# naver/panst3r

Hardware: AMD Instinct MI355X
Metric: frames/sec (whole node), N-view 512px panoptic inference (higher is better)
Workload: dtype f16

## Files before the change

### include/panst3r_hip.h

```cpp
#ifndef PANST3R_HIP_H
#define PANST3R_HIP_H
#include <stdint.h>
#ifdef __cplusplus
extern "C" {
#endif

#define PST_ABI_VERSION 20

#define PST_BF16 0
#define PST_F32  1
#define PST_F16  2
#define PST_X3H  4

int pst_abi_version(void);
const char* pst_last_error(void);

typedef struct pst_gemm_params {
  const void* A;  int64_t lda;
  const void* W;  int64_t ldw;
  void* C;        int64_t ldc;
  int32_t M, N, K;
  const float* bias;
  const float* gamma;
  const float* res;  int64_t ldr;
  int32_t res_mod;
  int32_t act;
  int32_t out_fp32;
  int32_t trans_out;
  int32_t grp_in, grp_out, grp_off;
  int32_t ps_p, ps_c, ps_h, ps_w;
  int32_t conv_c, conv_h, conv_w;
  const void* zeros;
  const int32_t* rope_pos; const float* rope_cs; int32_t rope_hd;
  int32_t rope_npos;
  int32_t res_bf16;
  int32_t kernel;
  int32_t batch;
  int64_t a_bs, w_bs, c_bs, bias_bs;
  int32_t dtype16;
  void* xcopy; int64_t ldxc;
  float* stats_out; int32_t stats_ld;
  const float* ln_stats; int32_t ln_groups; const float* ln_colsum; float ln_eps;
  int32_t x3_block;
} pst_gemm_params;

int pst_gemm(const pst_gemm_params* p, void* stream);
const char* pst_gemm_variant(const pst_gemm_params* p);
int pst_gemm_pair(const pst_gemm_params* a, const pst_gemm_params* b, void* stream);
const char* pst_gemm_pair_variant(const pst_gemm_params* a, const pst_gemm_params* b);
#define PST_TUNE_G256_PP 3
#define PST_TUNE_PAIR 4
#define PST_TUNE_DEEP_RING 8
#define PST_TUNE_PAIR_ATTN 7
#define PST_TUNE_ATTN_XCD 9
#define PST_TUNE_CUS 10
#define PST_TUNE_PAIR_DELAY 6
#define PST_TUNE_DEPHASE 11
#define PST_TUNE_PAIR_RES 5
int pst_tune(int knob, int value);

int pst_mask_head_supported(int Q, int P, int C);
int pst_mask_head(const void* E, int64_t lde, const void* F, int64_t f_view_stride, float* out, int64_t out_view_stride, int nviews, int Q, int P, int C,
                  int dtype16, void* stream);

typedef struct pst_attn_params {
  const void* Q;  int64_t q_bs, q_hs, q_rs;
  const void* K;  int64_t k_bs, k_hs, k_rs;
  const void* Vt; int64_t v_bs, v_hs, v_ds;
  void* O;        int64_t o_bs, o_hs, o_rs;
  const uint8_t* mask; int64_t m_bs, m_rs;
  int32_t B, H, Nq, Nk, hd;
  float scale;
  const void* zeros;
  int32_t nsplit;
  void* ws; int64_t ws_bytes;
  int32_t dtype16;
  int32_t prescaled;
} pst_attn_params;

int64_t pst_attn_workspace_bytes(int B, int H, int Nq, int hd, int nsplit);

int pst_attn_fwd(const pst_attn_params* p, void* stream);
const char* pst_attn_variant(const pst_attn_params* p);
int pst_attn_pair(const pst_attn_params* a, const pst_attn_params* b, void* stream);
const char* pst_attn_pair_variant(const pst_attn_params* a, const pst_attn_params* b);

int pst_layernorm(const void* x, int64_t ldx, int in_fp32, void* y, int64_t ldy, int out_fp32,
                  const float* gamma, const float* beta, int rows, int D, float eps,
                  int grp_in, int grp_out, int grp_off, void* stream);
int pst_layernorm_add(const void* x, int64_t ldx, int in_fp32, const float* add, int64_t ld_add, void* y, int64_t ldy,
                      int out_fp32, const float* gamma, const float* beta, int rows, int D, float eps,
                      int grp_in, int grp_out, int grp_off, void* stream);

int pst_token_embed(const int32_t* ids, int B, int L, const float* tok, int vocab, const float* pos, int npos, int D, float* out, int64_t ldo,
                    int32_t* status, void* stream);

int pst_rowstats(const void* x, int64_t ldx, int x_type, void* xcopy, int64_t ldxc, float* stats, int stats_ld, int rows, int D, int dtype16,
                 void* stream);

int pst_layernorm_add_batch(const void* x, int64_t ldx, int in_fp32, const float* add, int64_t ld_add, void* y, int64_t ldy,
                            int out_fp32, const float* gamma, const float* beta, int rows, int D, float eps,
                            int grp_in, int grp_out, int grp_off, int nbatch, int64_t x_bs, int64_t y_bs, int64_t w_bs,
                            void* stream);

int pst_split3(const float* x, int64_t ldx, void* out, int64_t ldo, int rows, int K, int dtype16, void* stream);

int pst_split_operand(const float* x, int64_t ldx, void* out, int64_t ldo, int rows, int K, int Kpad, int side, int dtype16, void* stream);
int pst_split2(const float* x, int64_t ldx, void* hi, void* lo, int64_t ldo, int rows, int K, int transpose, int dtype16, void* stream);
int pst_transpose_f32(const float* x, int64_t ldx, float* y, int64_t ldy, int rows, int cols, void* stream);
int pst_rope2d_split(const float* x, int64_t ld, const int32_t* pos, const float* cs, void* hi, void* lo, int64_t ldo, int rows, int nheads, int hd, int dtype16,
                     void* stream);
int pst_attn_x3(const pst_attn_params* p, const void* Q_lo, const void* K_lo, const void* Vt_lo, int out_type, int64_t out_block, void* stream);
const char* pst_attn_x3_variant(const pst_attn_params* p);

int pst_rope2d(void* x, int64_t ld, const int32_t* pos, const float* cs, int rows, int nheads, int hd, int dtype16,
               void* stream);

int pst_patchify(const float* img, void* out, int64_t ld, int nimg, int C, int H, int W, int p, int dtype16, void* stream);
int pst_dino_preprocess(const float* img, float* out, int nimg, int H, int W, int Ho, int Wo, void* stream);

int pst_image_prepare(const uint8_t* src, int Hs, int Ws, float* dst, int Hr, int Wr, int top, int left, int H, int W, void* stream);
int pst_patch_rows(const float* img, void* enc, int64_t ld_enc, void* dino, int64_t ld_dino, int nimg, int H, int W, int p_enc, int p_dino,
                   int dino_transposed, int dtype16, void* stream);

int pst_add_cast(const void* a, int64_t lda, int a_fp32, const void* b, int64_t ldb, int b_fp32, int b_mod,
                 void* y, int64_t ldy, int y_fp32, int rows, int D, void* stream);
int pst_l2norm_rows(const float* x, int64_t ldx, void* y, int64_t ldy, int rows, int D, float eps, int dtype16, void* stream);

int pst_mean4(const void* F, void* Fm, int nimg, int Hm, int Wm, int C, int dtype16, void* stream);
int pst_resize_bilinear(const void* F, void* Fd, int nimg, int Hs, int Ws, int Hd, int Wd, int C, int dtype16, void* stream);
int pst_attn_mask_from_logits(const float* logits, int64_t ldl, uint8_t* mask, int64_t ldm, int Q, int Nk,
                              void* stream);

#define PST_STATS_BLOCKS 128
int pst_loftup_guidance_gn(const float* img, const float* biases, const float* gamma, const float* beta, float eps,
                           float* scratch, float* stats, void* y, int64_t ldy, int nimg, int H, int W, int nf, int dtype16,
                           const float* mm_ext, void* stream);
int pst_loftup_minmax(const float* img, float* mm, int nimg, int H, int W, void* stream);
int pst_minmax_merge(const float* mm, const int32_t* scope, float* out, int nviews, void* stream);
int pst_groupnorm_stats(const void* x, int64_t ldx, int x_fp32, float* stats, int nimg, int P, int C, int G,
                        void* stream);
int pst_groupnorm_apply(const void* x, int64_t ldx, int x_fp32, const float* stats, const float* gamma,
                        const float* beta, void* y, int64_t ldy, int nimg, int P, int C, int G, float eps, int relu,
                        int dtype16, void* stream);
int pst_loftup_lr_pe(const float* biases, void* out, int64_t ld, int col0, int nimg, int h, int w, int dtype16, void* stream);

int pst_pp_scores(const float* logits, int Q, int Ncls, float cls_threshold, float temperature, float* scores,
                  int* labels, int* keep, void* stream);
int pst_pp_scores_softmax(const float* logits, int Q, int Ncls, float cls_threshold, float* scores, int* labels, int* keep, void* stream);
int pst_pp_sigmoid(const float* logits, const int* keep, float* probs, int Q, int P, void* stream);
int pst_pp_argmax(const float* probs, const float* scores, const int* keep, int Q, int Hm, int Wm, int H, int W,
                  float mask_threshold, int* best_q, float* best_m, int* cnt_orig, int* cnt_mask, void* stream);
int pst_pp_argmax_logits(const float* logits, const float* scores, const int* keep, int Q, int Hm, int Wm, int H, int W,
                         float mask_threshold, int* best_q, float* best_m, int* cnt_orig, int* cnt_mask, void* stream);
int pst_pp_select(const int* keep, int* cnt_orig, int* cnt_mask, int Q, double overlap_threshold, int* keep_out,
                  int* seg_id, void* stream);
int pst_pp_finalize(const int* best_q, const float* best_m, const int* seg_id, int n, float mask_threshold,
                    float void_confidence, int* pan, float* conf, void* stream);

int pst_qubo_upsample(const float* logits, float* probs, int Q, int hm, int wm, int H, int W, void* stream);
int64_t pst_qubo_workspace_floats(int Q, int64_t P);
int pst_qubo_overlap(const float* probs, int Q, int64_t P, float* ws, double* Wacc, void* stream);
int pst_qubo_argmax(const float* probs, const int* sel, int nsel, int64_t P, float* conf, int* inst, void* stream);

int pst_pointmap_activate(const float* raw, float* pts3d, float* pts3d_local, float* conf, int64_t npix, int mode, void* stream);
int pst_focal_weiszfeld(const float* pts3d_local, const float* pp, float* focal, int nviews, int H, int W, int iters, void* stream);
int pst_rigid_moments(const float* x, const float* y, const float* conf, double* out, int nviews, int npix, float weight_offset, void* stream);

int pst_retrieval_select(const float* x, int64_t ldx, const int32_t* in_off, const int32_t* out_off, int nviews, int maxT, int D, float* out, int64_t ldo,
                         int32_t* sel_idx, void* stream);
int pst_retrieval_assign(const void* x3, int64_t ldx, const void* c3, int64_t ldc, const float* cnorm, int n, int k, int K3, int m, int nsplit,
                         float* ws_dist, int32_t* ws_ids, int32_t* ids, float* dist, int dtype16, void* stream);
int pst_retrieval_aggregate(const float* x, int64_t ldx, const float* cent, int64_t ldc, const int32_t* member, const int32_t* gstart, const int32_t* gword,
                            int ngroups, int D, float* sums, uint32_t* bits, void* stream);
int pst_retrieval_scores(const int32_t* q_off, const int32_t* q_word, const uint32_t* q_bits, const int32_t* db_off, const int32_t* db_word,
                         const uint32_t* db_bits, int nq_views, int ndb_views, int max_q, int D, float alpha, float tau, float* S, void* stream);

typedef struct pst_cloud_view {
  const float* conf;
  const float* pts3d;
  const float* pts3d_local;
  const float* img;
  const int32_t* pan;
  int64_t offset;
  int32_t npix;
  int32_t first_wg;
  float c2w[12];
} pst_cloud_view;

int pst_cloud_count(const pst_cloud_view* views, int nviews, int nwg, float thr, int32_t* counts, void* stream);
int pst_cloud_scan(const int32_t* counts, int n, int32_t* base, void* stream);
int pst_cloud_compact(const pst_cloud_view* views, int nviews, int nwg, float thr, const int32_t* base, const float* colors, int ncolors, float w1, float w2,
                      float* points, float* points_local, float* rgb, int32_t* pan, float* colors_out, int64_t* index, void* stream);
int pst_cloud_segment_median(const float* points_local, const int32_t* pan, const int32_t* m_ptr, int64_t max_points, const int32_t* id2row, int ntab, int nseg,
                             int32_t* hist, uint32_t* prefix, int32_t* rank, int32_t* nan_cnt, int32_t* count, float* median, void* stream);

int pst_voxel_insert(const float* points, int64_t M, float inv, uint64_t* keys, int64_t capacity, int32_t* first, int32_t* point_slot, int32_t* status,
                     int merge, void* stream);
int pst_voxel_count(const int32_t* point_slot, const int32_t* first, int64_t M, int32_t* counts, void* stream);
int pst_voxel_rank(const int32_t* point_slot, const int32_t* first, int64_t M, const int32_t* base, int32_t* slot_rank, int32_t* first_row, void* stream);
int pst_voxel_accumulate(const float* points, const float* rgb, const int32_t* pan, int64_t M, float inv, const int32_t* point_slot,
                         const int32_t* slot_rank, const int32_t* id2row, int ntab, int32_t* cnt, uint64_t* sums, uint64_t* pair_keys, int32_t* pair_cnt,
                         int64_t capacity, int32_t* point_voxel, int32_t* status, int merge, void* stream);
int pst_voxel_vote(const uint64_t* pair_keys, const int32_t* pair_cnt, int64_t capacity, uint64_t* best, void* stream);
int pst_voxel_emit(const float* points, const int64_t* index, const int32_t* first_row, const int32_t* mv_ptr, int64_t max_voxels, float inv,
                   double voxel_size, const int32_t* cnt, const uint64_t* sums, const uint64_t* best, const float* colors, int ncolors, float w1, float w2,
                   float* out_points, float* out_rgb, int32_t* out_pan, float* out_colors, int32_t* out_votes, int64_t* out_first, void* stream);

#define PST_VCC_FULL 1
#define PST_VCC_DUPLICATE 2
#define PST_VCC_RANGE 4
// ... 110 lines not shown
```

### panst3r_amd/csrc/gemm.hip

```cpp
#include "common.h"
#include "../../include/panst3r_hip.h"

namespace pst {

int launch_gemm256(const pst_gemm_params& p, hipStream_t s);
int launch_gemm256p(const pst_gemm_params& p, hipStream_t s, int cus);
int gemm256p_pair_split(const pst_gemm_params& a, const pst_gemm_params& b, int cus, double separate_us, double* pair_us);
double gemm256p_single_us(const pst_gemm_params& p, int cus);
int launch_gemm256p_pair(const pst_gemm_params& a, const pst_gemm_params& b, hipStream_t s, int cus, int g0);
bool gemm256_persistent_ok(const pst_gemm_params& p);
int gemm256_persistent_class(const pst_gemm_params& p);
int gemm_f32_validate(const pst_gemm_params& p);
int launch_gemm_f32(const pst_gemm_params& p, hipStream_t s);
int rowstream_class(const pst_gemm_params& p);
int launch_rowstream(const pst_gemm_params& p, hipStream_t s, int cus);

constexpr int BK = 64;
constexpr int GROUP_M = 8;

template <int F>
__device__ __forceinline__ int perm_row(int row) {
  const int sub = row / (16 * F), rho = row - sub * (16 * F);
  const int f = rho >> 4, g = (rho >> 2) & 3, r = rho & 3;
  return sub * (16 * F) + g * (4 * F) + 4 * f + r;
// ... 323 lines not shown
    if (p.grp_in > 0) { quot = rem / p.grp_in; rem -= quot * p.grp_in; }
#pragma unroll
    for (int it = 0; it < BM / 8; ++it) {
      const int r = tid / nchf + it * rstepf;
      const int m = m0 + r;
      resv[it] = make_float4(0.f, 0.f, 0.f, 0.f);
      if (r < BM && m < p.M && nf < p.N) {
        const int orow = p.grp_in > 0 ? quot * p.grp_out + p.grp_off + rem : m;
        resv[it] = *(const float4*)(p.res + (int64_t)(p.res_mod > 0 ? (m % p.res_mod) : orow) * p.ldr + nf);
      }
      rem += rstepf;
      if (p.grp_in > 0) {
        while (rem >= p.grp_in) { rem -= p.grp_in; ++quot; }
      }
    }
  }
  if (TRANS) {
    bf16_t* Ct = (bf16_t*)p.C;
#pragma unroll
    for (int j = 0; j < FN; ++j) {
      const int n = n0 + wc * (16 * FN) + j * 16 + l16;
      if (n >= p.N) continue;
      const float b = p.bias ? p.bias[n] : 0.f;
      const int mb = m0 + wr * (16 * FM) + g * (4 * FM);
      bf16_t* dst = Ct + (int64_t)n * p.ldc + mb;
      const float cs = p.ln_stats ? p.ln_colsum[n] : 0.f;
      float v[4 * FM];
#pragma unroll
      for (int i = 0; i < FM; ++i)
#pragma unroll
        for (int r = 0; r < 4; ++r) {
          const float2 st = p.ln_stats ? lnst[wr * (16 * FM) + g * (4 * FM) + 4 * i + r] : make_float2(1.f, 0.f);
          float x = fmaf(acc[i][j][r], st.x, fmaf(st.y, cs, b));
          if (p.act == 2) x = fmaxf(x, 0.f);
          v[4 * i + r] = x;
        }
      if (p.act == 1) {
#pragma unroll
        for (int i = 0; i < FM; ++i) gelu_erf4(*(float (*)[4])(v + 4 * i));
      }
      if (mb + 4 * FM <= p.M && (((uintptr_t)dst) & 15) == 0) {
#pragma unroll
        for (int q = 0; q < FM / 2; ++q)
          *(uint4*)(dst + 8 * q) = make_uint4(H16<F16>::pack(v[8 * q], v[8 * q + 1]), H16<F16>::pack(v[8 * q + 2], v[8 * q + 3]),
                                              H16<F16>::pack(v[8 * q + 4], v[8 * q + 5]), H16<F16>::pack(v[8 * q + 6], v[8 * q + 7]));
      } else if (mb + 4 * FM <= p.M) {
#pragma unroll
        for (int q = 0; q < FM; ++q)
          *(uint2*)(dst + 4 * q) = make_uint2(H16<F16>::pack(v[4 * q], v[4 * q + 1]), H16<F16>::pack(v[4 * q + 2], v[4 * q + 3]));
      } else {
        for (int r = 0; r < 4 * FM && mb + r < p.M; ++r) dst[r] = H16<F16>::from_f(v[r]);
      }
    }
    return;
  }

  const bool f32o = p.out_fp32 != 0;
  const int pitch = BN * (f32o ? 4 : 2);
  const int nch = pitch >> 4;
  __syncthreads();
  {
    const int cb = wc * (16 * FN) + g * (4 * FN);
    float4 bias4[FN], gam4[FN], cs4[FN];
#pragma unroll
    for (int j = 0; j < FN; ++j) {
      const int n = min(n0 + cb + 4 * j, p.N - 4);
      bias4[j] = p.bias ? *(const float4*)(p.bias + n) : make_float4(0.f, 0.f, 0.f, 0.f);
      gam4[j] = p.gamma ? *(const float4*)(p.gamma + n) : make_float4(1.f, 1.f, 1.f, 1.f);
      cs4[j] = p.ln_stats ? *(const float4*)(p.ln_colsum + n) : make_float4(0.f, 0.f, 0.f, 0.f);
    }
    float2 lns[FM];
#pragma unroll
    for (int i = 0; i < FM; ++i) lns[i] = p.ln_stats ? lnst[wr * (16 * FM) + i * 16 + l16] : make_float2(1.f, 0.f);
#pragma unroll
    for (int i = 0; i < FM; ++i) {
      const int r = wr * (16 * FM) + i * 16 + l16;
      char* rowp = smem + r * pitch;
      const int key = r & (nch - 1);
#pragma unroll
      for (int j = 0; j < FN; ++j) {
        float v[4] = {fmaf(acc[i][j][0], lns[i].x, fmaf(lns[i].y, cs4[j].x, bias4[j].x)), fmaf(acc[i][j][1], lns[i].x, fmaf(lns[i].y, cs4[j].y, bias4[j].y)),
                      fmaf(acc[i][j][2], lns[i].x, fmaf(lns[i].y, cs4[j].z, bias4[j].z)), fmaf(acc[i][j][3], lns[i].x, fmaf(lns[i].y, cs4[j].w, bias4[j].w))};
        if (p.act == 1) {
          gelu_erf4(v);
        } else if (p.act == 2) {
#pragma unroll
          for (int q = 0; q < 4; ++q) v[q] = fmaxf(v[q], 0.f);
        }
        v[0] *= gam4[j].x; v[1] *= gam4[j].y; v[2] *= gam4[j].z; v[3] *= gam4[j].w;
        const int col = cb + 4 * j;
        if (f32o) *(float4*)(rowp + ((((col >> 2) ^ key)) << 4)) = make_float4(v[0], v[1], v[2], v[3]);
        else *(uint2*)(rowp + ((((col >> 3) ^ key)) << 4) + ((col & 4) << 1)) = make_uint2(H16<F16>::pack(v[0], v[1]), H16<F16>::pack(v[2], v[3]));
      }
    }
  }
  __syncthreads();
  if (f32o) row_phase<BM, BN, true, F16>(p, smem, tid, m0, n0, resv);
  else row_phase<BM, BN, false, F16>(p, smem, tid, m0, n0, resv);
}

static int g_cu_budget = 0;
static int num_cus() {
  if (g_cu_budget > 0) return g_cu_budget;
  static int cus = 0;
  if (cus == 0) {
    int dev = 0;
    hipDeviceProp_t prop;
    if (hipGetDevice(&dev) == hipSuccess && hipGetDeviceProperties(&prop, dev) == hipSuccess) cus = prop.multiProcessorCount;
    if (cus <= 0) cus = 256;
  }
  return cus;
}

template <int FM, int FN, bool TRANS, int NST, bool F16>
__global__ __launch_bounds__(256, 2) void gemm_kernel(const pst_gemm_params p, const int ntiles, const int tiles_m, const int tiles_n) {
  gemm_tile<FM, FN, TRANS, NST, F16>(p, ntiles, tiles_m, tiles_n, blockIdx.x, blockIdx.y);
}

template <int FM, int FN, int NST, bool F16>
__global__ __launch_bounds__(256, 2) void gemm_pair_kernel(const pst_gemm_params pa, const int na, const int tma, const int tna,
                                                           const pst_gemm_params pb, const int nb, const int tmb, const int tnb) {
  if ((int)blockIdx.x < na) gemm_tile<FM, FN, false, NST, F16>(pa, na, tma, tna, blockIdx.x, 0);
  else gemm_tile<FM, FN, true, NST, F16>(pb, nb, tmb, tnb, (int)blockIdx.x - na, 0);
}

template <int FM, int FN, int NST, bool F16>
static int launch_pair_t(const pst_gemm_params& a, const pst_gemm_params& b, hipStream_t s) {
  constexpr int BM = 32 * FM, BN = 32 * FN;
  const int tma = (a.M + BM - 1) / BM, tna = (a.N + BN - 1) / BN, tmb = (b.M + BM - 1) / BM, tnb = (b.N + BN - 1) / BN;
  const size_t lds = NST * (BM + BN) * 128 + BM * sizeof(float2);
  hipLaunchKernelGGL((gemm_pair_kernel<FM, FN, NST, F16>), dim3(tma * tna + tmb * tnb), dim3(256), lds, s, a, tma * tna, tma, tna, b, tmb * tnb, tmb, tnb);
  return check_launch("gemm_pair");
}

template <int FM, int FN, bool TRANS, int NST, bool F16>
static int launch_t(const pst_gemm_params& p, hipStream_t s) {
  constexpr int BM = 32 * FM, BN = 32 * FN;
  const int tiles_m = (p.M + BM - 1) / BM, tiles_n = (p.N + BN - 1) / BN;
  const int tiles = tiles_m * tiles_n;
  const size_t lds = NST * (BM + BN) * 128 + BM * sizeof(float2);
  if constexpr (NST > 4) {
    static unsigned long long attr_seen = 0;
    once_per_device(attr_seen, [] { (void)hipFuncSetAttribute((const void*)gemm_kernel<FM, FN, TRANS, NST, F16>, hipFuncAttributeMaxDynamicSharedMemorySize, NST * (BM + BN) * 128 + BM * (int)sizeof(float2)); });
  }
  hipLaunchKernelGGL((gemm_kernel<FM, FN, TRANS, NST, F16>), dim3(tiles, p.batch > 1 ? p.batch : 1), dim3(256), lds, s, p, tiles, tiles_m, tiles_n);
  return check_launch("gemm");
}

template <int FM, int FN, bool TRANS, int NST>
static int launch(const pst_gemm_params& p, hipStream_t s) {
  return p.dtype16 == DT_F16 ? launch_t<FM, FN, TRANS, NST, true>(p, s) : launch_t<FM, FN, TRANS, NST, false>(p, s);
}

}

static int gemm_validate(const pst_gemm_params* pp) {
  using namespace pst;
  if (!pp) { set_error("gemm: null params"); return PST_EINVAL; }
  const pst_gemm_params& p = *pp;
  if (p.dtype16 == DT_F32) {
    if (p.M <= 0 || p.N <= 0 || p.K <= 0 || !p.A || !p.W || !p.C) { set_error("gemm: bad shape / null operand"); return PST_EINVAL; }
    if (p.kernel != 0) { set_error("gemm (fp32 operands): kernel must be 0"); return PST_EINVAL; }
    return pst::gemm_f32_validate(p);
  }
  if (p.dtype16 != DT_BF16 && p.dtype16 != DT_F16) { set_error("gemm: dtype16 must be PST_BF16, PST_F16 or PST_F32"); return PST_EINVAL; }
  if (p.act < 0 || p.act > 2) {
    set_error("gemm: act %d not available with 16-bit operands (0 none, 1 GELU(erf), 2 ReLU; 3 = GELU(tanh) needs fp32 operands)", p.act); return PST_EINVAL;
  }
  if (p.kernel != 0 && p.kernel != 128 && p.kernel != 256) { set_error("gemm: kernel must be 0 (auto), 128 or 256"); return PST_EINVAL; }
  if (p.kernel == 256 && (p.conv_c > 0 || (p.trans_out && pst::gemm256_persistent_class(p) != 3))) {
    set_error("gemm: the 256x256 kernel has no conv mode, and trans_out only in its persistent class (16-bit, ldc %% 8 == 0, N %% 64 == 0)"); return PST_EINVAL;
  }
  if (p.M <= 0 || p.N <= 0 || p.K <= 0) { set_error("gemm: bad shape M=%d N=%d K=%d", p.M, p.N, p.K); return PST_EINVAL; }
  if (p.K % 64 || p.N % 4) { set_error("gemm: need K%%64==0 and N%%4==0 (K=%d N=%d)", p.K, p.N); return PST_EINVAL; }
  if (!p.A || !p.W || !p.C) { set_error("gemm: null operand"); return PST_EINVAL; }
  if ((((uintptr_t)p.A | (uintptr_t)p.W) & 15) || ((uintptr_t)p.C & (p.out_fp32 ? 15 : 7))) {
    set_error("gemm: A/W must be 16-byte aligned, C 8-byte (bf16) / 16-byte (fp32) aligned"); return PST_EINVAL;
  }
  if ((p.ldw % 8) || (p.conv_c == 0 && (p.lda % 8))) { set_error("gemm: lda/ldw must be multiples of 8"); return PST_EINVAL; }
  if (p.conv_c > 0 && (p.conv_c % 64 || p.K != 9 * p.conv_c || !p.zeros || p.M % (p.conv_h * p.conv_w))) {
    set_error("gemm: bad conv mode (conv_c=%d K=%d)", p.conv_c, p.K); return PST_EINVAL;
  }
  if (p.ps_p > 0 && ((p.ps_p * p.ps_c) % 4 || p.N != p.ps_p * p.ps_p * p.ps_c || p.M % (p.ps_h * p.ps_w) || p.res || p.grp_in)) {
    set_error("gemm: bad pixel-shuffle store (p=%d c=%d N=%d)", p.ps_p, p.ps_c, p.N); return PST_EINVAL;
  }
  if (p.trans_out && (p.out_fp32 || p.res || p.gamma || p.grp_in || p.ps_p || (p.ldc % 4))) {
    set_error("gemm: trans_out supports bf16 + bias/act only, ldc%%4==0"); return PST_EINVAL;
  }
  if (!p.trans_out && !p.ps_p && (p.ldc % 4)) { set_error("gemm: ldc must be a multiple of 4"); return PST_EINVAL; }
  if (p.rope_hd != 0 && (p.rope_hd != 64 || p.out_fp32 || p.trans_out || p.ps_p || p.N % 64 || !p.rope_pos || !p.rope_cs || p.res)) {
    set_error("gemm: fused RoPE needs head dim 64, bf16 plain output, N%%64==0, no residual"); return PST_EINVAL;
  }
  if (p.res && (p.ldr % (p.res_bf16 ? 8 : 4))) { set_error("gemm: ldr must be a multiple of 4 (fp32) / 8 (bf16)"); return PST_EINVAL; }
  if (p.res && p.res_bf16 && ((uintptr_t)p.res & 15)) { set_error("gemm: bf16 residual must be 16-byte aligned"); return PST_EINVAL; }
  if ((p.stats_out || p.xcopy) && (p.N % 64 || p.ps_p || p.trans_out || p.res_mod || p.batch > 1 || (p.stats_out && p.stats_ld < p.N / 64) ||
                                   (p.xcopy && (!p.out_fp32 || p.ldxc % 4 || ((uintptr_t)p.xcopy & 7))))) {
    set_error("gemm: LayerNorm-fold producer outputs need a plain row-major store with N%%64==0 (xcopy: fp32 C only)"); return PST_EINVAL;
  }
  if (p.ln_stats && (!p.ln_colsum || p.ln_groups <= 0 || p.conv_c || p.batch > 1 || !(p.ln_eps > 0.f))) {
    set_error("gemm: LayerNorm-fold consumer needs ln_colsum, ln_groups > 0, ln_eps > 0 (no conv / batch mode)"); return PST_EINVAL;
  }
  if (p.x3_block && (!p.out_fp32 || p.dtype16 != DT_F16 || p.x3_block < p.N || p.x3_block % 4 || p.ldc < 3 * (int64_t)p.x3_block || p.ldc % 4 || p.ps_p || p.trans_out || p.xcopy ||
                     p.stats_out || p.batch > 1 || ((uintptr_t)p.C & 7))) {
    set_error("gemm: the split store (x3_block) needs out_fp32, f16 operands, x3_block >= N, ldc >= 3 x3_block, a plain row-major store"); return PST_EINVAL;
  }
  if (p.batch > 1 && (p.gamma || p.res || p.conv_c || p.rope_hd || p.ps_p || p.grp_in || p.kernel == 256 || p.batch > 65535 ||
                      (p.a_bs | p.w_bs | p.c_bs) % 8 || p.bias_bs % 4)) {
    set_error("gemm: strided batch supports bias/act/trans_out only, strides multiples of 8 elements (batch=%d)", p.batch); return PST_EINVAL;
  }
  return PST_OK;
}

static int g_deep_ring = 4;
namespace pst { int gemm256_pp(int set); int gemm256p_dephase(int set); int gemm256p_pair_delay(int set); int attn_pair_enable(int set); int attn_xcd_order(int set); }

static int gemm_choice(const pst_gemm_params& p) {
  const long big_tiles = (long)((p.M + 127) / 128) * ((p.N + 127) / 128) * (p.batch > 1 ? p.batch : 1);
  const bool small = p.kernel == 0 && big_tiles < (p.K >= 2048 ? 176 : 256);
  const long tiles256 = (long)((p.M + 255) / 256) * ((p.N + 255) / 256);
  const bool fits32 = (int64_t)p.M * p.lda < (1ll << 31) && (int64_t)p.N * p.ldw < (1ll << 31);
  const bool one_round = tiles256 >= 176 && tiles256 <= 256;
  if (p.trans_out) {
    const bool p3 = pst::gemm256_persistent_class(p) == 3 && fits32 && p.batch <= 1 && (p.kernel == 256 || (p.kernel == 0 && (tiles256 >= 384 || one_round) && p.K >= 512));
    return p3 ? 2 : (small ? 0 : 1);
  }
  const bool shape256 = p.N % 256 == 0 && p.K >= 1024 && (p.N >= 2048 || p.K >= 2048) && tiles256 >= 3 * 256 - 64;
  const int pclass = pst::gemm256_persistent_class(p);
  const bool shape256p = (tiles256 >= 384 || one_round) && ((pclass == 1 && p.K >= 512) || (pclass == 2 && (p.K >= 2048 || (p.K >= 768 && tiles256 <= 512))));
  if (p.conv_c == 0 && fits32 && p.batch <= 1 && (p.kernel == 256 || (p.kernel == 0 && (shape256 || shape256p)))) return 2;
  return small ? 0 : 1;
}

extern "C" int pst_gemm(const pst_gemm_params* pp, void* stream) {
  using namespace pst;
  if (int rc = gemm_validate(pp)) return rc;
  const pst_gemm_params& p = *pp;
  hipStream_t s = (hipStream_t)stream;
  if (p.dtype16 == DT_F32) return launch_gemm_f32(p, s);
  if (rowstream_class(p)) return launch_rowstream(p, s, num_cus());
  const int c = gemm_choice(p);
  if (c == 2) return gemm256_persistent_ok(p) ? launch_gemm256p(p, s, num_cus()) : launch_gemm256(p, s);
  if (p.trans_out) return c == 0 ? launch<2, 2, true, 4>(p, s) : launch<4, 4, true, 2>(p, s);
  if (c == 0 && g_deep_ring > 4 && p.batch <= 1) {
    const long tiles = (long)((p.M + 63) / 64) * ((p.N + 63) / 64);
    if (tiles <= num_cus() && p.K >= 512) return g_deep_ring >= 8 ? launch<2, 2, false, 8>(p, s) : launch<2, 2, false, 6>(p, s);
  }
  return c == 0 ? launch<2, 2, false, 4>(p, s) : launch<4, 4, false, 2>(p, s);
}

static bool pair_fusable(const pst_gemm_params& a, const pst_gemm_params& b) {
  using namespace pst;
  if (a.dtype16 == DT_F32 || a.dtype16 != b.dtype16 || a.trans_out || !b.trans_out || a.batch > 1 || b.batch > 1 || a.kernel || b.kernel) return false;
  if (rowstream_class(a) || rowstream_class(b)) return false;
  return gemm_choice(a) == 0 && gemm_choice(b) == 0;
}

static int g_pair_res = 1;
static int g_pair = 1;
static int pair_split_256p(const pst_gemm_params& a, const pst_gemm_params& b) {
  using namespace pst;
  if (!g_pair || a.dtype16 == DT_F32 || a.dtype16 != b.dtype16 || a.batch > 1 || b.batch > 1 || a.kernel || b.kernel) return 0;
  if (rowstream_class(a) || rowstream_class(b)) return 0;
  const int cus = num_cus();
  double sep = 0.0;
  const pst_gemm_params* ps[2] = {&a, &b};
  for (const pst_gemm_params* p : ps) {
    const bool fits32 = (int64_t)p->M * p->lda < (1ll << 31) && (int64_t)p->N * p->ldw < (1ll << 31);
    if (gemm_choice(*p) == 2 && gemm256_persistent_ok(*p)) { sep += gemm256p_single_us(*p, cus); continue; }
    const long tiles256 = (long)((p->M + 255) / 256) * ((p->N + 255) / 256);
    if (!(g_pair_res && gemm256_persistent_class(*p) == 2 && fits32 && p->conv_c == 0 && p->K >= 1024 && tiles256 >= 128)) return 0;
    sep += 2.0 * p->M * p->N * p->K / 470e6;
  }
  return gemm256p_pair_split(a, b, cus, sep, nullptr);
}

extern "C" int pst_gemm_pair(const pst_gemm_params* pa, const pst_gemm_params* pb, void* stream) {
  using namespace pst;
  if (int rc = gemm_validate(pa)) return rc;
  if (int rc = gemm_validate(pb)) return rc;
  hipStream_t s = (hipStream_t)stream;
  if (const int g0 = pair_split_256p(*pa, *pb)) return launch_gemm256p_pair(*pa, *pb, s, num_cus(), g0);
  if (!pair_fusable(*pa, *pb)) {
    if (int rc = pst_gemm(pa, stream)) return rc;
    return pst_gemm(pb, stream);
  }
  return pa->dtype16 == DT_F16 ? launch_pair_t<2, 2, 4, true>(*pa, *pb, s) : launch_pair_t<2, 2, 4, false>(*pa, *pb, s);
}

extern "C" const char* pst_gemm_pair_variant(const pst_gemm_params* pa, const pst_gemm_params* pb) {
  if (gemm_validate(pa) || gemm_validate(pb)) return nullptr;
  if (pair_split_256p(*pa, *pb)) return "gemm256p2_kernel";
  return pair_fusable(*pa, *pb) ? "gemm_pair_kernel<2,2>" : "";
}

extern "C" int pst_tune(int knob, int value) {
  if (knob == PST_TUNE_G256_PP) return pst::gemm256_pp(value);
  if (knob == PST_TUNE_PAIR_RES) { const int prev = g_pair_res; g_pair_res = value != 0; return prev; }
  if (knob == PST_TUNE_PAIR_DELAY) return pst::gemm256p_pair_delay(value);
  if (knob == PST_TUNE_DEPHASE) return pst::gemm256p_dephase(value);
  if (knob == PST_TUNE_PAIR_ATTN) return pst::attn_pair_enable(value);
  if (knob == PST_TUNE_ATTN_XCD) return pst::attn_xcd_order(value);
  if (knob == PST_TUNE_DEEP_RING) { const int prev = g_deep_ring; if (value == 4 || value == 6 || value == 8) g_deep_ring = value; return prev; }
  if (knob == PST_TUNE_PAIR) { const int prev = g_pair; g_pair = value != 0; return prev; }
  if (knob == PST_TUNE_CUS) { const int prev = pst::g_cu_budget; if (value >= 0 && value <= 1024) pst::g_cu_budget = value; return prev; }
  return -1;
}

extern "C" const char* pst_gemm_variant(const pst_gemm_params* pp) {
  if (gemm_validate(pp)) return nullptr;
  if (pp->dtype16 == pst::DT_F32) return "gemm_f32_kernel";
  if (pst::rowstream_class(*pp)) return "rowgemm384_kernel";
  const int c = gemm_choice(*pp);
  if (pp->trans_out && c != 2) return c == 0 ? "gemm_kernel<2,2,true>" : "gemm_kernel<4,4,true>";
  return c == 2 ? (pst::gemm256_persistent_ok(*pp) ? "gemm256p_kernel" : "gemm256_kernel") : (c == 0 ? "gemm_kernel<2,2,false>" : "gemm_kernel<4,4,false>");
}
```

### panst3r_amd/hip.py

```python
import ctypes as C
import os
import torch

_HERE = os.path.dirname(os.path.abspath(__file__))
LIB_PATH = os.environ.get('PST_LIB') or os.path.join(_HERE, 'lib', 'libpanst3r_hip.so')
ABI_VERSION = 20
STATS_BLOCKS = 128
_lib = None

i32, i64, f32, vp = C.c_int32, C.c_int64, C.c_float, C.c_void_p


class GemmParams(C.Structure):
    _fields_ = [('A', vp), ('lda', i64), ('W', vp), ('ldw', i64), ('C', vp), ('ldc', i64),
                ('M', i32), ('N', i32), ('K', i32),
                ('bias', vp), ('gamma', vp), ('res', vp), ('ldr', i64), ('res_mod', i32),
                ('act', i32), ('out_fp32', i32), ('trans_out', i32),
                ('grp_in', i32), ('grp_out', i32), ('grp_off', i32),
                ('ps_p', i32), ('ps_c', i32), ('ps_h', i32), ('ps_w', i32),
                ('conv_c', i32), ('conv_h', i32), ('conv_w', i32), ('zeros', vp), ('rope_pos', vp), ('rope_cs', vp), ('rope_hd', i32), ('rope_npos', i32), ('res_bf16', i32), ('kernel', i32),
                ('batch', i32), ('a_bs', i64), ('w_bs', i64), ('c_bs', i64), ('bias_bs', i64), ('dtype16', i32),
                ('xcopy', vp), ('ldxc', i64), ('stats_out', vp), ('stats_ld', i32), ('ln_stats', vp), ('ln_groups', i32), ('ln_colsum', vp), ('ln_eps', f32), ('x3_block', i32)]


class AttnParams(C.Structure):
    _fields_ = [('Q', vp), ('q_bs', i64), ('q_hs', i64), ('q_rs', i64),
                ('K', vp), ('k_bs', i64), ('k_hs', i64), ('k_rs', i64),
                ('Vt', vp), ('v_bs', i64), ('v_hs', i64), ('v_ds', i64),
                ('O', vp), ('o_bs', i64), ('o_hs', i64), ('o_rs', i64),
                ('mask', vp), ('m_bs', i64), ('m_rs', i64),
                ('B', i32), ('H', i32), ('Nq', i32), ('Nk', i32), ('hd', i32),
                ('scale', f32), ('zeros', vp), ('nsplit', i32), ('ws', vp), ('ws_bytes', i64), ('dtype16', i32), ('prescaled', i32)]


class CloudView(C.Structure):
    _fields_ = [('conf', vp), ('pts3d', vp), ('pts3d_local', vp), ('img', vp), ('pan', vp), ('offset', i64), ('npix', i32), ('first_wg', i32), ('c2w', f32 * 12)]


_CODES = {'i': C.c_int, 'l': C.c_int64, 'u': C.c_uint64, 'f': C.c_float, 'd': C.c_double, 'p': vp, 's': C.c_char_p,
          'G': C.POINTER(GemmParams), 'A': C.POINTER(AttnParams)}
SIGNATURES = {
    'pst_abi_version': 'i:', 'pst_last_error': 's:', 'pst_gemm': 'i:Gp', 'pst_gemm_variant': 's:G', 'pst_gemm_pair': 'i:GGp', 'pst_gemm_pair_variant': 's:GG',
    'pst_tune': 'i:ii', 'pst_mask_head_supported': 'i:iii', 'pst_mask_head': 'i:plplpliiiiip', 'pst_attn_workspace_bytes': 'l:iiiii', 'pst_attn_fwd': 'i:Ap',
    'pst_attn_variant': 's:A', 'pst_attn_pair': 'i:AAp', 'pst_attn_pair_variant': 's:AA', 'pst_layernorm': 'i:pliplippiifiiip',
    'pst_layernorm_add': 'i:pliplplippiifiiip', 'pst_token_embed': 'i:piipipiiplpp', 'pst_rowstats': 'i:pliplpiiiip',
    'pst_layernorm_add_batch': 'i:pliplplippiifiiiilllp', 'pst_split3': 'i:plpliiip', 'pst_split_operand': 'i:plpliiiiip', 'pst_split2': 'i:plppliiiip',
    'pst_transpose_f32': 'i:plpliip', 'pst_rope2d_split': 'i:plppppliiiip', 'pst_attn_x3': 'i:Apppilp', 'pst_attn_x3_variant': 's:A',
    'pst_rope2d': 'i:plppiiiip', 'pst_patchify': 'i:ppliiiiiip', 'pst_dino_preprocess': 'i:ppiiiiip', 'pst_image_prepare': 'i:piipiiiiiip',
    'pst_patch_rows': 'i:pplpliiiiiiip', 'pst_add_cast': 'i:plipliipliiip', 'pst_l2norm_rows': 'i:plpliifip', 'pst_mean4': 'i:ppiiiiip',
    'pst_resize_bilinear': 'i:ppiiiiiiip', 'pst_attn_mask_from_logits': 'i:plpliip', 'pst_loftup_guidance_gn': 'i:ppppfpppliiiiipp',
    'pst_loftup_minmax': 'i:ppiiip', 'pst_minmax_merge': 'i:pppip', 'pst_groupnorm_stats': 'i:plipiiiip', 'pst_groupnorm_apply': 'i:plippppliiiifiip',
    'pst_loftup_lr_pe': 'i:ppliiiiip', 'pst_pp_scores': 'i:piiffpppp', 'pst_pp_scores_softmax': 'i:piifpppp', 'pst_pp_sigmoid': 'i:pppiip',
    'pst_pp_argmax': 'i:pppiiiiifppppp', 'pst_pp_argmax_logits': 'i:pppiiiiifppppp', 'pst_pp_select': 'i:pppidppp', 'pst_pp_finalize': 'i:pppiffppp',
    'pst_qubo_upsample': 'i:ppiiiiip', 'pst_qubo_workspace_floats': 'l:il', 'pst_qubo_overlap': 'i:pilppp', 'pst_qubo_argmax': 'i:ppilppp',
    'pst_pointmap_activate': 'i:pppplip', 'pst_focal_weiszfeld': 'i:pppiiiip', 'pst_rigid_moments': 'i:ppppiifp', 'pst_retrieval_select': 'i:plppiiiplpp',
    'pst_retrieval_assign': 'i:plplpiiiiippppip', 'pst_retrieval_aggregate': 'i:plplpppiippp', 'pst_retrieval_scores': 'i:ppppppiiiiffpp',
    'pst_cloud_count': 'i:piifpp', 'pst_cloud_scan': 'i:pipp', 'pst_cloud_compact': 'i:piifppiffppppppp', 'pst_cloud_segment_median': 'i:ppplpiippppppp',
    'pst_qubo_anneal_max_n': 'i:', 'pst_qubo_anneal': 'i:piiifffuppppp',
    'pst_voxel_insert': 'i:plfplpppip', 'pst_voxel_count': 'i:pplpp', 'pst_voxel_rank': 'i:pplpppp', 'pst_voxel_accumulate': 'i:ppplfpppipppplppip',
    'pst_voxel_vote': 'i:pplpp', 'pst_voxel_emit': 'i:pppplfdppppiffppppppp',
    'pst_render_max_radius': 'i:', 'pst_render_splat': 'i:plpiiifiipip', 'pst_render_resolve': 'i:pllppppppppp',
    'pst_consist_depth': 'i:ppiilfipp', 'pst_consist_count': 'i:pppiilfippppp',
    'pst_mesh_lane_pixels': 'i:', 'pst_mesh_raster': 'i:plplpiiiffppplip', 'pst_mesh_resolve': 'i:piiiplplpfpppppp', 'pst_mesh_area_count': 'i:pilpiipp',
    'pst_mesh_area_apply': 'i:pilpiipipp',
    'pst_pq_count': 'i:pplpipipiiipip', 'pst_pq_match': 'i:piiipppppppp',
    'pst_vcc_cells': 'i:ppplfpp', 'pst_vcc_build': 'i:pplpplppp', 'pst_vcc_link': 'i:pplpplippp', 'pst_vcc_flatten': 'i:ppplppppppip', 'pst_vcc_count': 'i:plpp',
    'pst_vcc_rank': 'i:pplpppppppppppppp', 'pst_vcc_votes': 'i:pppplppliipplpp', 'pst_vcc_apply': 'i:pppplippiffpppp',
    'pst_surface_rows': 'i:pllpp', 'pst_surface_count': 'i:ppiipfpp', 'pst_surface_emit': 'i:ppiipfpppppp', 'pst_surface_link': 'i:pllpppp',
    'pst_surface_components': 'i:pllppppp', 'pst_surface_keep_count': 'i:pplipp', 'pst_surface_keep_emit': 'i:ppppplippppp',
    'pst_mesh_sample_count': 'i:plplfipppp', 'pst_mesh_sample_emit': 'i:plplpllppppppp',
    'pst_nn_insert': 'i:plfplpppp', 'pst_nn_scatter': 'i:plpppppp', 'pst_nn_query': 'i:plplffplpppipppp',
    'pst_icp_chunk': 'i:', 'pst_icp_step': 'i:plffffffffffffplffplpppipppppp',
    'pst_meshdist_count': 'i:plplfpppp', 'pst_meshdist_insert': 'i:plplfplplpppp', 'pst_meshdist_scatter': 'i:ppllpppppp',
    'pst_meshdist_query': 'i:plplplffplppplippppp',
    'pst_plane_icp_step': 'i:plfffffffffffffffplplffplppplipppppp',
}
EXPORTS = list(SIGNATURES)


def lib():
    global _lib
    if _lib is not None:
        return _lib
    if not os.path.exists(LIB_PATH):
        raise RuntimeError('libpanst3r_hip.so not found at %s -- run `python -m panst3r_amd.build` (hipcc, gfx950). '
                           'The HIP path has no fallback.' % LIB_PATH)
    L = C.CDLL(LIB_PATH)
    for name, sig in SIGNATURES.items():
        ret, args = sig.split(':')
        fn = getattr(L, name)
        fn.restype, fn.argtypes = _CODES[ret], [_CODES[c] for c in args]
    if L.pst_abi_version() != ABI_VERSION:
        raise RuntimeError('libpanst3r_hip.so ABI %d != expected %d; rebuild' % (L.pst_abi_version(), ABI_VERSION))
    _lib = L
    return L


TUNE_G256_PP, TUNE_PAIR, TUNE_PAIR_RES, TUNE_PAIR_DELAY, TUNE_PAIR_ATTN, TUNE_DEEP_RING, TUNE_ATTN_XCD, TUNE_CUS, TUNE_DEPHASE = 3, 4, 5, 6, 7, 8, 9, 10, 11


def tune(knob, value):
    return int(lib().pst_tune(int(knob), int(value)))


def _stream():
    return torch.cuda.current_stream().cuda_stream


def _ptr(t):
    return t.data_ptr() if t is not None else None


def _call(what, *args):
    rc = getattr(lib(), what)(*args, _stream())
    if rc != 0:
        raise RuntimeError('%s failed (%d): %s' % (what, rc, lib().pst_last_error().decode()))


H16 = (torch.bfloat16, torch.float16)
FMT = H16 + (torch.float32,)
_TC = {torch.bfloat16: 0, torch.float32: 1, torch.float16: 2}


def _tc(t):
    return _TC[t.dtype]


def _same16(*ts):
    dts = {t.dtype for t in ts if t is not None and t.dtype in H16}
    if len(dts) != 1:
        raise RuntimeError('16-bit operands of one call must share one format, got %s' % sorted(str(d) for d in dts))
    return _TC[dts.pop()]


def _fmt(*ts):
    dts = {t.dtype for t in ts if t is not None}
    if len(dts) != 1 or next(iter(dts)) not in FMT:
        raise RuntimeError('the operands of this call must share one of the formats bf16 / f16 / f32, got %s' % sorted(str(d) for d in dts))
    return _TC[dts.pop()]


def _dev(t, *dtypes):
    if not t.is_cuda:
        raise RuntimeError('panst3r_amd HIP op got a %s tensor: the HIP path runs on the GPU only (no CPU fallback)' % t.device)
    if dtypes and t.dtype not in dtypes:
        raise RuntimeError('unexpected dtype %s (want %s)' % (t.dtype, dtypes))
    return t


class KernelTimer:

    def __init__(self):
        self.records = []

    def bracket(self, name, flops, tag=None):
        a, b = torch.cuda.Event(enable_timing=True), torch.cuda.Event(enable_timing=True)
        self.records.append((name, flops, a, b, tag))
        return a, b

    def by_tag(self):
        torch.cuda.synchronize()
        out = {}
        for name, flops, a, b, tag in self.records:
            d = out.setdefault((name, tag), dict(launches=0, ms=0.0, flops=0.0))
            d['launches'] += 1
            d['ms'] += a.elapsed_time(b)
            d['flops'] += flops
        return out

    def summary(self):
        torch.cuda.synchronize()
        out = {}
        for name, flops, a, b, tag in self.records:
            d = out.setdefault(name, dict(launches=0, ms=0.0, flops=0.0, bytes=0.0))
            d['launches'] += 1
            d['ms'] += a.elapsed_time(b)
            d['flops'] += flops
            if tag and tag[0] == 'bytes':
                d['bytes'] += tag[1]
        return out


TIMER = None

MAXABS = None
_STAGE = ['']
F16_MAX = 65504.0


class _Ctx:
    def __init__(self, enter, leave):
        self._enter, self._leave = enter, leave

    def __enter__(self):
        return self._enter()

    def __exit__(self, *exc):
        self._leave()
        return False


def maxabs_telemetry():
    def enter():
        global MAXABS
        MAXABS = {}
        return MAXABS

    def leave():
        global MAXABS
        MAXABS = None
    return _Ctx(enter, leave)


def stage(name):
    return _Ctx(lambda: _STAGE.append(name), lambda: _STAGE.pop())


def note_maxabs(t, what):
    if MAXABS is None or t is None or not torch.is_tensor(t) or t.dtype not in H16 or t.numel() == 0:
        return
    if torch.cuda.is_current_stream_capturing():
        raise RuntimeError('hip.maxabs_telemetry() needs eager launches (it synchronises after every producer)')
    v = float(torch.amax(t.abs()).float())
    if v != v:
        v = float('inf')
    key = (_STAGE[-1], what)
    MAXABS[key] = max(MAXABS.get(key, 0.0), v)


def maxabs_report(log, top=None):
    rows = sorted(((k[0], k[1], v, v / F16_MAX) for k, v in log.items()), key=lambda r: -r[2])
    return rows[:top] if top else rows


def _esz(t):
    return t.element_size()


def hbm_timed(name, nbytes):
    def deco(fn):
        def wrapped(*a, **k):
            return _timed(name, 0.0, ('bytes', float(nbytes(*a, **k))) if TIMER is not None else None, fn, *a, **k)
        wrapped.__name__, wrapped.__doc__ = fn.__name__, fn.__doc__
        return wrapped
    return deco


def _timed(name, flops, tag, fn, *a, **k):
    if TIMER is None:
        return fn(*a, **k)
    ev = TIMER.bracket(name() if callable(name) else name, flops, tag)
# ... 1417 lines not shown
```

Measured before the change: 333.5.

## Add 128x384 full-width GEMM kernel for N=384 16-bit projections

Adds a dedicated 512-thread GEMM kernel that tiles 128 rows by the full 384-column width, so each A row block is loaded once and reused across all output columns. It uses double-buffered LDS staging with an explicit fragment-read/MFMA software pipeline and a swizzled LDS epilogue for coalesced stores. It is selected by default only for plain bias/activation GEMMs with N=384, K>=576 and enough M to fill the CUs, replacing the generic 128x128 tile path. The cost is one block per CU with large LDS use, plus a new tuning knob to disable or force it.

```diff
diff --git a/include/panst3r_hip.h b/include/panst3r_hip.h
--- a/include/panst3r_hip.h
+++ b/include/panst3r_hip.h
@@ -57,6 +57,7 @@
 #define PST_TUNE_PAIR_DELAY 6
 #define PST_TUNE_DEPHASE 11
 #define PST_TUNE_PAIR_RES 5
+#define PST_TUNE_WIDE384 12
 int pst_tune(int knob, int value);
 
 int pst_mask_head_supported(int Q, int P, int C);
diff --git a/panst3r_amd/csrc/gemm.hip b/panst3r_amd/csrc/gemm.hip
--- a/panst3r_amd/csrc/gemm.hip
+++ b/panst3r_amd/csrc/gemm.hip
@@ -499,6 +499,186 @@
   return p.dtype16 == DT_F16 ? launch_t<FM, FN, TRANS, NST, true>(p, s) : launch_t<FM, FN, TRANS, NST, false>(p, s);
 }
 
+constexpr int W384_BM = 128, W384_BN = 384, W384_BUF = (W384_BM + W384_BN) * 128;
+
+template <bool F16>
+__global__ __launch_bounds__(512, 1) void gemm_wide384_kernel(const pst_gemm_params p, const int ntiles) {
+  constexpr int FM = 4, FN = 6;
+  extern __shared__ __attribute__((aligned(16))) char smem[];
+  const int tid = threadIdx.x, lane = tid & 63;
+  const int wave = __builtin_amdgcn_readfirstlane(tid >> 6);
+  const int wr = wave >> 2, wc = wave & 3;
+  const int g = lane >> 4, l16 = lane & 15;
+  const int m0 = xcd_remap(blockIdx.x, ntiles) * W384_BM;
+  const bf16_t* Ap = (const bf16_t*)p.A;
+  const bf16_t* Wp = (const bf16_t*)p.W;
+
+  const int sw = ((tid & 7) ^ ((tid >> 4) & 7)) << 3;
+  int a_base[2], a_yx[2], b_base[FN];
+#pragma unroll
+  for (int j = 0; j < 2; ++j) {
+    const int m = min(m0 + j * 64 + (tid >> 3), p.M - 1);
+    if (p.conv_c > 0) {
+      const int hw = p.conv_h * p.conv_w;
+      const int img = m / hw, r = m - img * hw;
+      const int y = r / p.conv_w;
+      a_yx[j] = (y << 16) | (r - y * p.conv_w);
+      a_base[j] = img * hw * p.conv_c;
+    } else {
+      a_yx[j] = 0;
+      a_base[j] = m * p.lda;
+    }
+  }
+#pragma unroll
+  for (int j = 0; j < FN; ++j) b_base[j] = perm_row<FN>(j * 64 + (tid >> 3)) * p.ldw + sw;
+
+  int st_k0 = 0, st_tap = 0, st_c0 = 0;
+  auto stage = [&](int buf) {
+    char* a_dst = smem + buf * W384_BUF + wave * 1024;
+    char* b_dst = a_dst + W384_BM * 128;
+    if (p.conv_c > 0) {
+      const int dy = st_tap / 3 - 1, dx = st_tap - (st_tap / 3) * 3 - 1;
+#pragma unroll
+      for (int j = 0; j < 2; ++j) {
+        const int yy = (a_yx[j] >> 16) + dy, xx = (a_yx[j] & 0xffff) + dx;
+        const bool ok = (yy >= 0) & (yy < p.conv_h) & (xx >= 0) & (xx < p.conv_w);
+        const bf16_t* s = ok ? Ap + (a_base[j] + (yy * p.conv_w + xx) * p.conv_c + st_c0 + sw) : (const bf16_t*)p.zeros + sw;
+        glds16(s, a_dst + j * 8192);
+      }
+      st_c0 += BK;
+      if (st_c0 == p.conv_c) { st_c0 = 0; ++st_tap; }
+    } else {
+#pragma unroll
+      for (int j = 0; j < 2; ++j) glds16(Ap + (a_base[j] + st_k0 + sw), a_dst + j * 8192);
+    }
+#pragma unroll
+    for (int j = 0; j < FN; ++j) glds16(Wp + (b_base[j] + st_k0), b_dst + j * 8192);
+    st_k0 += BK;
+  };
+
+  f32x4 acc[FM][FN];
+#pragma unroll
+  for (int i = 0; i < FM; ++i)
+#pragma unroll
+    for (int j = 0; j < FN; ++j) acc[i][j] = f32x4{0.f, 0.f, 0.f, 0.f};
+
+  const int key = (l16 >> 1) & 7;
+  const int a_off = (wr * (16 * FM) + l16) * 128 + ((g ^ key) << 4);
+  const int b_off = W384_BM * 128 + (wc * (16 * FN) + l16) * 128 + ((g ^ key) << 4);
+  const uint32_t lds0 = lds_addr(smem);
+
+  bf16x8 af[2][FM], bfv[2][FN];
+#pragma unroll
+  for (int i = 0; i < FM; ++i) af[1][i] = bf16x8{};
+#pragma unroll
+  for (int j = 0; j < FN; ++j) bfv[1][j] = bf16x8{};
+  auto read_frags = [&](auto kk, uint32_t buf) {
+    static_for<0, FN>([&](auto j) { ds_read128<j * 2048>(bfv[kk][j], buf + (uint32_t)(b_off ^ (kk << 6))); });
+    static_for<0, FM>([&](auto i) { ds_read128<i * 2048>(af[kk][i], buf + (uint32_t)(a_off ^ (kk << 6))); });
+  };
+  auto mma = [&](auto kk, auto i) {
+#pragma unroll
+    for (int j = 0; j < FN; ++j) acc[i][j] = H16<F16>::mfma(bfv[kk][j], af[kk][i], acc[i][j]);
+    __builtin_amdgcn_sched_barrier(0);
+  };
+  constexpr std::integral_constant<int, 0> c0{};
+  constexpr std::integral_constant<int, 1> c1{};
+
+  const int nk = p.K / BK;
+  stage(0);
+  if (nk > 1) { stage(1); asm volatile("s_waitcnt vmcnt(8)" ::: "memory"); }
+  else wait_vm0();
+  __builtin_amdgcn_s_barrier();
+  auto step = [&](int kt, auto first) {
+    const uint32_t buf = lds0 + (uint32_t)((kt & 1) * W384_BUF);
+    read_frags(c0, buf);
+    if constexpr (!first) {
+      __builtin_amdgcn_s_setprio(1);
+      static_for<0, FM>([&](auto i) { mma(c1, i); });
+      __builtin_amdgcn_s_setprio(0);
+    }
+    lgkm_wait<FM - 1>(af[0][0]);
+    static_for<0, FN>([&](auto j) { lds_tie(bfv[0][j]); });
+    read_frags(c1, buf);
+    __builtin_amdgcn_s_setprio(1);
+    static_for<0, FM>([&](auto i) {
+      if constexpr (i > 0) lgkm_wait<FM - 1 - i + FM + FN>(af[0][i]);
+      mma(c0, i);
+    });
+    __builtin_amdgcn_s_setprio(0);
+    lgkm_wait<0>(af[1][0]);
+    static_for<1, FM>([&](auto i) { lds_tie(af[1][i]); });
+    static_for<0, FN>([&](auto j) { lds_tie(bfv[1][j]); });
+    wait_vm0();
+    __builtin_amdgcn_s_barrier();
+    if (kt + 2 < nk) stage(kt & 1);
+  };
+  step(0, c1);
+  for (int kt = 1; kt < nk; ++kt) step(kt, c0);
+  __builtin_amdgcn_s_setprio(1);
+  static_for<0, FM>([&](auto i) { mma(c1, i); });
+  __builtin_amdgcn_s_setprio(0);
+
+  constexpr int pitch = W384_BN * 2;
+  {
+    const int cb = wc * (16 * FN) + g * (4 * FN);
+    float4 bias4[FN];
+#pragma unroll
+    for (int j = 0; j < FN; ++j) bias4[j] = p.bias ? *(const float4*)(p.bias + cb + 4 * j) : make_float4(0.f, 0.f, 0.f, 0.f);
+    const float2 lns = make_float2(1.f, 0.f);
+    const float cs = 0.f;
+#pragma unroll
+    for (int i = 0; i < FM; ++i) {
+      const int r = wr * (16 * FM) + i * 16 + l16;
+      char* rowp = smem + r * pitch;
+      const int rkey = r & 15;
+#pragma unroll
+      for (int j = 0; j < FN; ++j) {
+        float v[4] = {fmaf(acc[i][j][0], lns.x, fmaf(lns.y, cs, bias4[j].x)), fmaf(acc[i][j][1], lns.x, fmaf(lns.y, cs, bias4[j].y)),
+                      fmaf(acc[i][j][2], lns.x, fmaf(lns.y, cs, bias4[j].z)), fmaf(acc[i][j][3], lns.x, fmaf(lns.y, cs, bias4[j].w))};
+        if (p.act == 1) {
+          gelu_erf4(v);
+        } else if (p.act == 2) {
+#pragma unroll
+          for (int q = 0; q < 4; ++q) v[q] = fmaxf(v[q], 0.f);
+        }
+        const int col = cb + 4 * j;
+        *(uint2*)(rowp + (((col >> 3) ^ rkey) << 4) + ((col & 4) << 1)) = make_uint2(H16<F16>::pack(v[0], v[1]), H16<F16>::pack(v[2], v[3]));
+      }
+    }
+  }
+  __syncthreads();
+  constexpr int nch = pitch >> 4;
+#pragma unroll
+  for (int it = 0; it < W384_BM * nch / 512; ++it) {
+    const int idx = it * 512 + tid;
+    const int r = idx / nch, c = idx - r * nch;
+    const int m = m0 + r;
+    if (m >= p.M) continue;
+    const uint4 val = *(const uint4*)(smem + r * pitch + ((c ^ (r & 15)) << 4));
+    *(uint4*)((char*)p.C + ((int64_t)m * p.ldc + c * 8) * 2) = val;
+  }
+}
+
+static bool wide384_class(const pst_gemm_params& p) {
+  if (p.N != W384_BN || p.dtype16 == DT_F32 || p.out_fp32 || p.kernel != 0 || p.batch > 1 || p.trans_out || p.ps_p || p.grp_in || p.x3_block) return false;
+  if (p.res || p.res_mod || p.gamma || p.rope_hd || p.stats_out || p.xcopy || p.ln_stats) return false;
+  if ((p.ldc & 7) || ((uintptr_t)p.C & 15) || ((uintptr_t)p.bias & 15)) return false;
+  return (int64_t)p.M * (p.conv_c > 0 ? p.conv_c : p.lda) < (1ll << 31) && (int64_t)p.N * p.ldw < (1ll << 31);
+}
+
+static int launch_wide384(const pst_gemm_params& p, hipStream_t s) {
+  const int tiles = (p.M + W384_BM - 1) / W384_BM;
+  static unsigned long long attr_seen = 0;
+  once_per_device(attr_seen, [] {
+    (void)hipFuncSetAttribute((const void*)gemm_wide384_kernel<true>, hipFuncAttributeMaxDynamicSharedMemorySize, 2 * W384_BUF);
+    (void)hipFuncSetAttribute((const void*)gemm_wide384_kernel<false>, hipFuncAttributeMaxDynamicSharedMemorySize, 2 * W384_BUF);
+  });
+  if (p.dtype16 == DT_F16) hipLaunchKernelGGL((gemm_wide384_kernel<true>), dim3(tiles), dim3(512), 2 * W384_BUF, s, p, tiles);
+  else hipLaunchKernelGGL((gemm_wide384_kernel<false>), dim3(tiles), dim3(512), 2 * W384_BUF, s, p, tiles);
+  return check_launch("gemm_wide384");
+}
+
 }
 
 static int gemm_validate(const pst_gemm_params* pp) {
@@ -578,6 +758,13 @@
   return small ? 0 : 1;
 }
 
+static int g_wide384 = 1;
+static bool wide384_choice(const pst_gemm_params& p) {
+  if (g_wide384 == 0 || !pst::wide384_class(p)) return false;
+  if (g_wide384 == 2) return true;
+  return gemm_choice(p) == 1 && p.K >= 576 && p.M >= 2 * pst::W384_BM * pst::num_cus();
+}
+
 extern "C" int pst_gemm(const pst_gemm_params* pp, void* stream) {
   using namespace pst;
   if (int rc = gemm_validate(pp)) return rc;
@@ -585,6 +772,7 @@
   hipStream_t s = (hipStream_t)stream;
   if (p.dtype16 == DT_F32) return launch_gemm_f32(p, s);
   if (rowstream_class(p)) return launch_rowstream(p, s, num_cus());
+  if (wide384_choice(p)) return launch_wide384(p, s);
   const int c = gemm_choice(p);
   if (c == 2) return gemm256_persistent_ok(p) ? launch_gemm256p(p, s, num_cus()) : launch_gemm256(p, s);
   if (p.trans_out) return c == 0 ? launch<2, 2, true, 4>(p, s) : launch<4, 4, true, 2>(p, s);
@@ -649,6 +837,7 @@
   if (knob == PST_TUNE_ATTN_XCD) return pst::attn_xcd_order(value);
   if (knob == PST_TUNE_DEEP_RING) { const int prev = g_deep_ring; if (value == 4 || value == 6 || value == 8) g_deep_ring = value; return prev; }
   if (knob == PST_TUNE_PAIR) { const int prev = g_pair; g_pair = value != 0; return prev; }
+  if (knob == PST_TUNE_WIDE384) { const int prev = g_wide384; if (value >= 0 && value <= 2) g_wide384 = value; return prev; }
   if (knob == PST_TUNE_CUS) { const int prev = pst::g_cu_budget; if (value >= 0 && value <= 1024) pst::g_cu_budget = value; return prev; }
   return -1;
 }
@@ -657,6 +846,7 @@
   if (gemm_validate(pp)) return nullptr;
   if (pp->dtype16 == pst::DT_F32) return "gemm_f32_kernel";
   if (pst::rowstream_class(*pp)) return "rowgemm384_kernel";
+  if (wide384_choice(*pp)) return "gemm_wide384_kernel";
   const int c = gemm_choice(*pp);
   if (pp->trans_out && c != 2) return c == 0 ? "gemm_kernel<2,2,true>" : "gemm_kernel<4,4,true>";
   return c == 2 ? (pst::gemm256_persistent_ok(*pp) ? "gemm256p_kernel" : "gemm256_kernel") : (c == 0 ? "gemm_kernel<2,2,false>" : "gemm_kernel<4,4,false>");
diff --git a/panst3r_amd/hip.py b/panst3r_amd/hip.py
--- a/panst3r_amd/hip.py
+++ b/panst3r_amd/hip.py
@@ -97,6 +97,7 @@
 
 
 TUNE_G256_PP, TUNE_PAIR, TUNE_PAIR_RES, TUNE_PAIR_DELAY, TUNE_PAIR_ATTN, TUNE_DEEP_RING, TUNE_ATTN_XCD, TUNE_CUS, TUNE_DEPHASE = 3, 4, 5, 6, 7, 8, 9, 10, 11
+TUNE_WIDE384 = 12
 
 
 def tune(knob, value):
```

Result: no change. 336.8, median of 6 (+1.0%).
